# idthanm/env_build

Measured on AMD Instinct MI355X. Metric: env-steps/s (batched rollout) at N_env x N_veh; achieved HBM GB/s vs peak, higher is better.
Workload: dtype f32

## Files before the change

env_build_amd/csrc/eb_rollout.hip:

```cpp
#include <type_traits>

#include "eb_device.h"
#include "eb_kernels.h"

#pragma clang fp contract(off)

namespace eb {

typedef float f2u __attribute__((ext_vector_type(2), aligned(4)));
typedef float v2f __attribute__((ext_vector_type(2)));
EB_DEV v2f fma2(v2f a, v2f b, v2f c) { return __builtin_elementwise_fma(a, b, c); }

template <typename ST> struct Stored;
template <> struct Stored<float> {
    static EB_DEV f4u load4(const float* p) { return *reinterpret_cast<const f4u*>(p); }
    static EB_DEV float load1(const float* p) { return *p; }
    static EB_DEV void store4(float* p, f4u v) { *reinterpret_cast<f4u*>(p) = v; }
    static EB_DEV void store1(float* p, float v) { *p = v; }
    static EB_DEV float round(float v) { return v; }
    static EB_DEV void store4_wt(float* p, f4u v) { asm volatile("global_store_dwordx4 %0, %1, off sc1\n\ts_nop 1" :: "v"(p), "v"(v) : "memory"); }
    static EB_DEV void store1_wt(float* p, float v) { asm volatile("global_store_dword %0, %1, off sc1" :: "v"(p), "v"(v) : "memory"); }
};
typedef _Float16 h4u __attribute__((ext_vector_type(4), aligned(2)));
template <> struct Stored<_Float16> {
    static EB_DEV f4u load4(const _Float16* p) {
        const h4u h = *reinterpret_cast<const h4u*>(p);
        return f4u{(float)h.x, (float)h.y, (float)h.z, (float)h.w};
    }
    static EB_DEV float load1(const _Float16* p) { return (float)*p; }
    static EB_DEV void store4(_Float16* p, f4u v) {
        *reinterpret_cast<h4u*>(p) = h4u{(_Float16)v.x, (_Float16)v.y, (_Float16)v.z, (_Float16)v.w};
    }
    static EB_DEV void store1(_Float16* p, float v) { *p = (_Float16)v; }
    static EB_DEV float round(float v) { return (float)(_Float16)v; }
    static EB_DEV void store4_wt(_Float16* p, f4u v) {
        typedef unsigned u2v __attribute__((ext_vector_type(2)));
        const u2v bits = __builtin_bit_cast(u2v, h4u{(_Float16)v.x, (_Float16)v.y, (_Float16)v.z, (_Float16)v.w});
        asm volatile("global_store_dwordx2 %0, %1, off sc1" :: "v"(p), "v"(bits) : "memory");
    }
    static EB_DEV void store1_wt(_Float16* p, float v) {
        const unsigned bits = __builtin_bit_cast(unsigned short, (_Float16)v);
        asm volatile("global_store_short %0, %1, off sc1" :: "v"(p), "v"(bits) : "memory");
    }
};

EB_DEV void lds_barrier() { asm volatile("s_waitcnt lgkmcnt(0)\n\ts_barrier" ::: "memory"); }
typedef __attribute__((address_space(3))) int lds_int;
EB_DEV void lds_publish(int* flag, int value) {
    asm volatile("s_waitcnt lgkmcnt(0)" ::: "memory");
    *(volatile lds_int*)flag = value;
}
EB_DEV void lds_wait_until(int* flag, int value) {
    while (*(volatile lds_int*)flag != value) __builtin_amdgcn_s_sleep(2);
    asm volatile("" ::: "memory");
}

template <int CTRL, int ROW_MASK>
EB_DEV double dpp_f64(double v) {
    const unsigned long long b = __builtin_bit_cast(unsigned long long, v);
    const unsigned lo = (unsigned)__builtin_amdgcn_update_dpp(0, (int)(unsigned)b, CTRL, ROW_MASK, 0xf, false);
    const unsigned hi = (unsigned)__builtin_amdgcn_update_dpp(0, (int)(unsigned)(b >> 32), CTRL, ROW_MASK, 0xf, false);
    return __builtin_bit_cast(double, ((unsigned long long)hi << 32) | lo);
}
EB_DEV double wave_sum_f64(double v) {
    v += dpp_f64<0x111, 0xf>(v);
    v += dpp_f64<0x112, 0xf>(v);
    v += dpp_f64<0x114, 0xf>(v);
    v += dpp_f64<0x118, 0xf>(v);
    v += dpp_f64<0x142, 0xa>(v);
    v += dpp_f64<0x143, 0xc>(v);
    return v;
}
template <int CTRL, int ROW_MASK>
EB_DEV float dpp_max_f32(float v) {
    const float o = __builtin_bit_cast(float, __builtin_amdgcn_update_dpp(0, __builtin_bit_cast(int, v), CTRL, ROW_MASK, 0xf, false));
    return o > v ? o : v;
}
EB_DEV float wave_max_f32(float v) {
    v = dpp_max_f32<0x111, 0xf>(v);
    v = dpp_max_f32<0x112, 0xf>(v);
    v = dpp_max_f32<0x114, 0xf>(v);
    v = dpp_max_f32<0x118, 0xf>(v);
    v = dpp_max_f32<0x142, 0xa>(v);
    v = dpp_max_f32<0x143, 0xc>(v);
    return v;
}

EB_DEV void acc_record(double* recs, bool act, int lane, float v_r, float v_t, float v_p) {
    const double s_r = wave_sum_f64(act ? (double)v_r : 0.0);
    const double s_t = wave_sum_f64(act ? (double)v_t : 0.0);
    const double s_p = wave_sum_f64(act ? (double)v_p : 0.0);
    const unsigned long long any = __builtin_amdgcn_ballot_w64(act && v_p > 0.0f);
    if (lane == 63) {
        typedef double d2v __attribute__((ext_vector_type(2)));
        d2v* rec = reinterpret_cast<d2v*>(recs + (size_t)ACC_RECORD_DOUBLES * blockIdx.x);
        rec[0] = d2v{s_r, s_t};
        rec[1] = d2v{s_p, __builtin_bit_cast(double, any)};
    }
}

EB_DEV unsigned agent_load_u32(const unsigned* p) {
    unsigned v;
    asm volatile("global_load_dword %0, %1, off sc1\n\ts_waitcnt vmcnt(0)" : "=v"(v) : "v"(p) : "memory");
    return v;
}
EB_DEV unsigned long long agent_load_u64(const void* p) {
    unsigned long long v;
    asm volatile("global_load_dwordx2 %0, %1, off sc1\n\ts_waitcnt vmcnt(0)" : "=v"(v) : "v"(p) : "memory");
    return v;
}
EB_DEV void agent_store_u32(unsigned* p, unsigned v) { asm volatile("global_store_dword %0, %1, off sc1" :: "v"(p), "v"(v) : "memory"); }
EB_DEV void agent_add_u32(unsigned* p, unsigned v) { asm volatile("global_atomic_add %0, %1, off sc1" :: "v"(p), "v"(v) : "memory"); }

template <typename ST>
struct FusedHot {
    const ST* obs_in;
    ST* obs_out;
    int n_env, obs_dim, n_veh, envs_per_tile;
    unsigned nv_magic;
    int do_rewards;
    double* acc_rec;
    const unsigned char* turn;
    long long t_entry;
};
constexpr int HOT_REWARDS = 1, HOT_PRIO = 2;

template <typename ST>
EB_DEV int env_of_item(const FusedHot<ST>& H, int item) {
    return H.nv_magic ? (int)__umulhi((unsigned)item, H.nv_magic) : item;
}

#define EB_MARK(A, row, i) do { if ((A).trace && (threadIdx.x & 63) == 0) (A).trace[(size_t)(row) * 8 + (i)] = wall_clock64(); } while (0)
#define EB_MARK_PLACE(A, row) do { if ((A).trace && (threadIdx.x & 63) == 0) (A).trace[(size_t)(row) * 8 + 7] = \
    ((long long)__builtin_amdgcn_s_getreg((31 << 11) | 20) << 32) | (unsigned)__builtin_amdgcn_s_getreg((31 << 11) | 4); } while (0)

constexpr int QCAP = 160;
constexpr int TAPE_QCAP = 192;

template <int PRE = 3, bool COARSE = true>
EB_DEV int closest_cell_index(const FusedArgs& A, const float* xy10, const float* phi10, int p, int roff, float px, float py,
                              float& rx, float& ry, float& rphi) {
    const float* xy = xy10 + 2 * roff;
    const float* ph = phi10 + roff;
    const float fx = (px - A.gx0) * CELL_INV, fy = (py - A.gy0) * CELL_INV;
    unsigned c = 0xffffffffu;
    if (fx >= 0.0f && fx < (float)A.gnx && fy >= 0.0f && fy < (float)A.gny) c = A.cells[(p * A.gny + (int)fy) * A.gnx + (int)fx];
    if (c == 0xffffffffu) {
        int r_first = 0, r_last = 1 << 30;
        if constexpr (COARSE) {
            const PathTables& pt = *A.dt;
            int lo, hi, lo2, hi2;
            const int how = coarse_cell_ranges(pt, p, px, py, lo, hi, lo2, hi2);
            if (how == 1) return closest_in_ranges(xy, ph, lo, hi, lo2, hi2, px, py, rx, ry, rphi);
            if (how == 2) { r_first = lo; r_last = hi; }
        }
        const int n = p == 0 ? A.red_len[0] : p == 1 ? A.red_len[1] : A.red_len[2];
        const int bi = closest_reduced_index(reinterpret_cast<const float2*>(xy), A.rad_all + 32 * p, n, px, py, r_first, r_last);
        rx = xy[2 * bi]; ry = xy[2 * bi + 1]; rphi = ph[bi];
        return bi;
    }
    if (PRE > 0 && A.scan_one_trip) return closest_in_range<0>(xy, ph, (int)(c & 0xffffu), (int)(c >> 16), px, py, rx, ry, rphi);
    return closest_in_range<PRE>(xy, ph, (int)(c & 0xffffu), (int)(c >> 16), px, py, rx, ry, rphi);
}

template <int RW, int RPT>
struct FusedSmem {
    static constexpr int ITEMS = RW * 64 * RPT;
    float4 ego[64];
    unsigned char turn[64];
    unsigned long long mask[64];
    float2 pen[ITEMS];
    v2f qxy[RW][QCAP];
    v2f qsc[RW][QCAP];
    int qitem[RW][QCAP];
    int ego_ready;
    int waves_done;
};

template <int TASK, int RW, int RPT, typename ST>
EB_DEV void env_wave(const FusedHot<ST>& H, const FusedArgs& A, FusedSmem<RW, RPT>& S, int e0, int nE) {
    const int lane = threadIdx.x;
    const int D = H.obs_dim, NV = H.n_veh;
    const bool act = lane < nE;
    const int e = act ? lane : 0, ge = e0 + e;
    const ST* hin = H.obs_in + (size_t)ge * D;
    ST* hout = H.obs_out + (size_t)ge * D;

    const f4u h0 = Stored<ST>::load4(hin), h1 = Stored<ST>::load4(hin + 4);
    const float h8 = Stored<ST>::load1(hin + 8);
    const f2u araw = *reinterpret_cast<const f2u*>(A.actions + 2 * (size_t)ge);
    int p = A.path_id;
    if (A.training) {
        const int pr = A.ref_idx[ge];
        p = (pr >= 0 && pr < A.n_paths) ? pr : -1;
    }
    float sh_prev = 0.0f;
    if (A.shield_punish && !A.shield_first && act) sh_prev = A.shield_punish[ge];
    const int trow = blockIdx.x * (RW + 1);
    if (lane == 0) { S.ego_ready = 0; S.waves_done = 0; }
    lds_barrier();
    EB_MARK(A, trow, 0);
    EB_MARK_PLACE(A, trow);
    const bool do_rewards = (H.do_rewards & HOT_REWARDS) != 0;
    const float st[6] = {h0.x, h0.y, h0.z, h0.w, h1.x, h1.y};
    const float phi_rad = deg2rad(st[5]);
    float es, ec;
    sincos_det(phi_rad, es, ec);
    if (do_rewards) {
        S.ego[lane] = make_float4(st[3], st[4], es, ec);
        S.mask[lane] = 0ull;
        lds_publish(&S.ego_ready, 1);
        EB_MARK(A, trow, 1);
    }

    float steer, a_x;
    if (A.actions_raw) action_transform(araw.x, araw.y, steer, a_x);
    else { steer = araw.x; a_x = araw.y; }
    if (act && A.scaled_actions) *reinterpret_cast<f2u*>(A.scaled_actions + 2 * (size_t)ge) = f2u{steer, a_x};
    float rew = 0.0f;
    if (act && do_rewards) {
        const float punish_steer = -sq(steer), punish_a_x = -sq(a_x);
        const float punish_yaw_rate = -sq(st[2]);
        const float devi_y = -sq(h1.z);
        const float devi_phi = -sq(deg2rad(h1.w));
        const float devi_v = -sq(h8);
        rew = 0.05f * devi_v + 0.8f * devi_y + 30.0f * devi_phi + 0.02f * punish_yaw_rate +
              5.0f * punish_steer + 0.05f * punish_a_x;
        A.out5[ge] = rew;
    }
    float nx[6];
    f_xu_core(st, steer, a_x, TAU10, phi_rad, es, ec, nx);
    nx[0] = __builtin_fminf(__builtin_fmaxf(nx[0], 0.0f), 35.0f);
    float t0 = 0.0f, t1 = 0.0f, t2 = 0.0f;
    if (p >= 0) {
        const int roff = p == 0 ? A.red_off[0] : p == 1 ? A.red_off[1] : A.red_off[2];
        EB_MARK(A, trow, 2);
        float rx = 0.0f, ry = 0.0f, rphi = 0.0f;
        constexpr int SCAN_PRE = RW * RPT >= 32 ? 0 : 3;
        const int bi = closest_cell_index<SCAN_PRE>(A, A.xy10, A.phi10, p, roff, nx[3], nx[4], rx, ry, rphi);
        t0 = two2one<TASK>(nx[3], nx[4], rx, ry);
        if (A.trace) { asm volatile("" :: "v"(t0)); EB_MARK(A, trow, 3); }
        t1 = deal_with_phi_diff(nx[5] - rphi);
        t2 = nx[0] - EXP_V;
        if (A.n_future > 0 && act) {
            const PathTables& pt = *A.dt;
            const int len = pt.len[p];
            ST* otrk = hout + 9;
            int cur = bi * 10;
            for (int k = 0; k < A.n_future; ++k) {
                cur += 80;
                if (cur >= len - 2) cur = len - 2;
                const int fi = clamp_index(cur, len);
                Stored<ST>::store1(otrk + 3 * k, pt.x[p][fi] - nx[3]);
                Stored<ST>::store1(otrk + 3 * k + 1, pt.y[p][fi] - nx[4]);
                Stored<ST>::store1(otrk + 3 * k + 2, deal_with_phi_diff(nx[5] - pt.phi[p][fi]));
            }
        }
    } else if (A.n_future > 0 && act) {
        ST* otrk = hout + 9;
        for (int c = 0; c < 3 * A.n_future; ++c) Stored<ST>::store1(otrk + c, 0.0f);
    }
    if (act) {
        Stored<ST>::store4(hout, f4u{nx[0], nx[1], nx[2], nx[3]});
        Stored<ST>::store4(hout + 4, f4u{nx[4], nx[5], t0, t1});
        Stored<ST>::store1(hout + 8, t2);
    }
    EB_MARK(A, trow, 4);
    if (!do_rewards) return;
    float road_t = 0.0f, road_r = 0.0f;
    road_terms<TASK>(st[3] + LWS * ec, st[4] + LWS * es, road_t, road_r);
    road_terms<TASK>(st[3] - LWS * ec, st[4] - LWS * es, road_t, road_r);
    lds_wait_until(&S.waves_done, RW);
    EB_MARK(A, trow, 5);

    float pun_t = 0.0f, pun_r = 0.0f;
    if (act) {
        float a35 = 0.0f, a25 = 0.0f;
        unsigned long long m = S.mask[lane];
        while (m) {
            const int jj = __ffsll((long long)m) - 1;
            m &= m - 1;
            const float2 ps = S.pen[lane * NV + jj];
            a35 += ps.x;
            a25 += ps.y;
        }
        const size_t n = (size_t)H.n_env;
        pun_t = a35 + road_t;
        pun_r = a25 + road_r;
        A.out5[n + ge] = pun_t;
        A.out5[2 * n + ge] = pun_r;
        A.out5[3 * n + ge] = a25;
        A.out5[4 * n + ge] = road_r;
        if (A.shield_punish) {
            const float pacc = sh_prev + (A.shield_row == 3 ? a25 : pun_r);
            A.shield_punish[ge] = pacc;
            if (A.shield_last) A.shield_safe[ge] = pacc > 0.0f ? 0 : 1;
        }
    }
    if (H.acc_rec && A.acc_final) {
        acc_record(H.acc_rec, act, lane, rew, pun_t, pun_r);
        const float dy = __builtin_fabsf(Stored<ST>::round(t0));
        const double s_dy = wave_sum_f64(act ? (double)dy : 0.0);
        const float m_dy = wave_max_f32(act && dy > 0.0f ? dy : 0.0f);
        if (lane == 63) {
            typedef double d2v __attribute__((ext_vector_type(2)));
            reinterpret_cast<d2v*>(A.acc_final)[blockIdx.x] = d2v{s_dy, (double)m_dy};
        }
    }
    EB_MARK(A, trow, 6);
}

template <typename SM, typename ST>
EB_DEV void queue_terms(const FusedHot<ST>& H, SM& S, const float4* ego, int item, float x, float y, float vs, float vc) {
    const int e2 = env_of_item(H, item), j2 = item - e2 * H.n_veh;
    const float4 eg = ego[e2];
    float t35[4], t25[4];
    const float4 pts = make_float4(eg.x + LWS * eg.w, eg.y + LWS * eg.z, eg.x - LWS * eg.w, eg.y - LWS * eg.z);
    veh2veh_terms(pts, x, y, vs, vc, t35, t25);
    const float p35 = ((t35[0] + t35[1]) + t35[2]) + t35[3];
    const float p25 = ((t25[0] + t25[1]) + t25[2]) + t25[3];
    if (p35 != 0.0f) {
        S.pen[item] = make_float2(p35, p25);
        atomicOr(&S.mask[e2], 1ull << j2);
    }
}
template <typename SM, typename ST>
EB_DEV void queue_pass(const FusedHot<ST>& H, SM& S, const float4* ego, int w, int lane, int base, int n) {
    if (lane < n) {
        const v2f vxy = S.qxy[w][base + lane];
        float vs, vc;
        sincos_det(deg2rad(S.qphi[w][base + lane]), vs, vc);
        queue_terms(H, S, ego, S.qitem[w][base + lane], vxy.x, vxy.y, vs, vc);
    }
}
template <typename SM, typename ST>
EB_DEV void queue_pass_sc(const FusedHot<ST>& H, SM& S, const float4* ego, int w, int lane, int base, int n) {
    if (lane < n) {
        const v2f vxy = S.qxy[w][base + lane], sc = S.qsc[w][base + lane];
        queue_terms(H, S, ego, S.qitem[w][base + lane], vxy.x, vxy.y, sc.x, sc.y);
    }
}


template <int TASK, int RW, int RPT, bool FAST, int PF, typename ST>
EB_DEV void record_wave(const FusedHot<ST>& H, const FusedArgs& A, FusedSmem<RW, RPT>& S, int e0, int nE) {
    constexpr int RL = RW * 64;
    const int rtid = threadIdx.x - 64, w = rtid >> 6, lane = rtid & 63;
    const int NV = H.n_veh, D = H.obs_dim, HD = D - 4 * NV;
    const int items = nE * NV;
    const ST* tin = H.obs_in + (size_t)e0 * D;
    ST* tout = H.obs_out + (size_t)e0 * D;
    const int e_first = env_of_item(H, rtid), j_first = rtid - e_first * NV;
    const int epk = RL / NV;
    const int off_first = 4 * rtid + (e_first + 1) * HD, off_step = 4 * RL + epk * HD;
    auto item_of = [&](int k) { return k * RL + rtid; };
    auto env_of = [&](int k) { return FAST ? e_first + k * epk : env_of_item(H, item_of(k)); };
    auto off_of = [&](int k) { return FAST ? off_first + k * off_step : 4 * item_of(k) + (env_of(k) + 1) * HD; };

    static_assert(PF >= 1 && PF <= RPT, "record loads in flight per lane");
    const int turn_code = H.turn[lane];
    f4u rec[PF];
    const bool full_tile = items == RL * RPT;
    auto load_records = [&](auto full_tag) {
        constexpr bool FULL = decltype(full_tag)::value;
#pragma unroll
        for (int k = 0; k < PF; ++k) {
            const bool valid = FULL || item_of(k) < items;
            rec[k] = Stored<ST>::load4(tin + (valid ? off_of(k) : 4 * (items - 1) + nE * HD));
            if (!valid) rec[k].x = 1e30f;
        }
    };
    if (full_tile) load_records(std::true_type{}); else load_records(std::false_type{});
    const bool acc_prev = w == 0 && H.acc_rec && A.prev_out5;
    float pv_r = 0.0f, pv_t = 0.0f, pv_p = 0.0f;
    if (acc_prev && lane < nE) {
        const size_t n = (size_t)H.n_env;
        const float* po = A.prev_out5 + e0 + lane;
        pv_r = po[0]; pv_t = po[n]; pv_p = po[2 * n];
    }
    const int trow = blockIdx.x * (RW + 1) + 1 + w;
    lds_barrier();
    EB_MARK(A, trow, 0);
    EB_MARK_PLACE(A, trow);
    if (A.trace && lane == 0) A.trace[(size_t)trow * 8 + 6] = H.t_entry;
    const bool do_rewards = (H.do_rewards & HOT_REWARDS) != 0;
    const bool by_progress = (H.do_rewards & HOT_PRIO) != 0;
    S.turn[lane] = (unsigned char)turn_code;
    const TurnC tc_lane = turn_consts(S.turn[FAST ? j_first : 0]);
    const SinCosK SK = sincos_consts();

    int qn = 0;
    auto drain = [&]() {
        for (int base = 0; base < qn; base += 64) queue_pass_sc(H, S, S.ego, w, lane, base, min(64, qn - base));
        qn = 0;
    };
    auto near_test = [&](int item, const v2f eg, const f4u r, const v2f sc) {
        const v2f d = v2f{r.x, r.y} - eg;
        const v2f d2 = d * d;
        const bool near = d2.x + d2.y < 40.5f;
        const unsigned long long b = __builtin_amdgcn_ballot_w64(near);
        if (b) {
            if (near) {
                const int pos = (int)__builtin_amdgcn_mbcnt_hi((unsigned)(b >> 32), __builtin_amdgcn_mbcnt_lo((unsigned)b, (unsigned)qn));
                S.qxy[w][pos] = v2f{r.x, r.y};
                S.qsc[w][pos] = sc;
                S.qitem[w][pos] = item;
            }
            qn += __popcll(b);
        }
    };
    if (do_rewards) {
        lds_wait_until(&S.ego_ready, 1);
        EB_MARK(A, trow, 3);
    }
    const bool test_near = do_rewards;
    int k_late = test_near ? RPT : 0;
    auto main_loop = [&](auto full_tag) {
        constexpr bool FULL = decltype(full_tag)::value;
        v2f egoxy[RPT];
        if (test_near) {
#pragma unroll
            for (int k = 0; k < RPT; ++k) {
                const int item = k * RL + rtid;
                const int env = FAST ? e_first + k * epk : env_of_item(H, item);
                egoxy[k] = *reinterpret_cast<const v2f*>(&S.ego[(FULL || item < items) ? env : 0]);
            }
        }
#pragma unroll
        for (int k = 0; k < RPT; ++k) {
            int k_item = k * RL, k_env = k * epk, k_off = k * off_step;
            asm volatile("" : "+s"(k_item), "+s"(k_env), "+s"(k_off));
            const int item = k_item + rtid;
            const int env = FAST ? e_first + k_env : env_of_item(H, item);
            const int off = FAST ? off_first + k_off : 4 * item + (env + 1) * HD;
            const bool valid = FULL || item < items;
            const TurnC tc = FAST ? tc_lane : turn_consts(S.turn[valid ? item - env * NV : 0]);
            float sn, cs;
            if ((k * 4) % RPT == 0 && by_progress)
                switch (3 - (k * 4) / RPT) {
                    case 3: __builtin_amdgcn_s_setprio(3); break;
                    case 2: __builtin_amdgcn_s_setprio(2); break;
                    case 1: __builtin_amdgcn_s_setprio(1); break;
                    default: __builtin_amdgcn_s_setprio(0); break;
                }
            const f4u nv = predict_record_tc<ST>(rec[k % PF], tc, SK, sn, cs);
            if (k < k_late) {
                near_test(item, egoxy[k], rec[k % PF], v2f{sn, cs});
                if (qn > QCAP - 64) k_late = k + 1;
            }
            if (k + PF < RPT) {
                const bool v2 = FULL || item_of(k + PF) < items;
                rec[k % PF] = Stored<ST>::load4(tin + (v2 ? off_of(k + PF) : 4 * (items - 1) + nE * HD));
                if (!v2) rec[k % PF].x = 1e30f;
            }
            if (valid) Stored<ST>::store4(reinterpret_cast<ST*>(reinterpret_cast<char*>(tout) + (unsigned)off * (unsigned)sizeof(ST)), nv);
            if (k == 0) EB_MARK(A, trow, 1);
            if (k == RPT - 1) EB_MARK(A, trow, 2);
            if (k & 1) __builtin_amdgcn_sched_barrier(0);
        }
    };
    if (full_tile) main_loop(std::true_type{}); else main_loop(std::false_type{});
    if (!do_rewards) return;
    if (by_progress) __builtin_amdgcn_s_setprio(0);
    if (test_near && k_late < RPT) {
        for (int k = k_late; k < RPT; ++k) {
            drain();
            const bool valid = item_of(k) < items;
            f4u r = Stored<ST>::load4(tin + (valid ? off_of(k) : 4 * (items - 1) + nE * HD));
            if (!valid) r.x = 1e30f;
            float sn, cs;
            sincos_det(deg2rad(r.w), sn, cs);
            near_test(item_of(k), *reinterpret_cast<const v2f*>(&S.ego[valid ? env_of(k) : 0]), r, v2f{sn, cs});
        }
    }
    EB_MARK(A, trow, 4);
    drain();
    asm volatile("s_waitcnt lgkmcnt(0)" ::: "memory");
    if (lane == 0) atomicAdd(&S.waves_done, 1);
    if (acc_prev) {
        asm volatile("" : "+v"(pv_r), "+v"(pv_t), "+v"(pv_p));
        acc_record(A.prev_rec, lane < nE, lane, pv_r, pv_t, pv_p);
    }
    EB_MARK(A, trow, 5);
}

template <int RW, int RPT>
struct TapeSmem {
    static constexpr int ITEMS = RW * 64 * RPT;
    float4 ego[2][64];
    unsigned char turn[64];
    unsigned long long mask[64];
    float2 pen[ITEMS];
    v2f qxy[RW][TAPE_QCAP];
    float qphi[RW][TAPE_QCAP];
    int qitem[RW][TAPE_QCAP];
    int ego_ready;
    int waves_done;
    int pub_done;
    int abort;
};
EB_DEV bool lds_wait_or_abort(int* flag, int value, int* abort) {
    while (*(volatile lds_int*)flag < value) {
        if (*(volatile lds_int*)abort) return false;
        __builtin_amdgcn_s_sleep(2);
    }
    asm volatile("" ::: "memory");
    return true;
}

struct GateSmem {
    f2u act[2][64];
    float out5[2][5][64];
    float head[2][9][64];
    int bi[2][64];
    int act_ready;
    int out_ready;
    int sent;
};

template <typename ST, bool WT>
EB_DEV void store_head_row(const FusedArgs& A, ST* row, const float (&hv)[9], int bi, int p) {
    auto s4 = [&](ST* q, f4u v) { if (WT) Stored<ST>::store4_wt(q, v); else Stored<ST>::store4(q, v); };
    auto s1 = [&](ST* q, float v) { if (WT) Stored<ST>::store1_wt(q, v); else Stored<ST>::store1(q, v); };
    s4(row, f4u{hv[0], hv[1], hv[2], hv[3]});
    s4(row + 4, f4u{hv[4], hv[5], hv[6], hv[7]});
    s1(row + 8, hv[8]);
    ST* otrk = row + 9;
    if (p >= 0) {
        const PathTables& pt = *A.dt;
        const int len = pt.len[p];
        int cur = bi * 10;
        for (int k = 0; k < A.n_future; ++k) {
            cur += 80;
            if (cur >= len - 2) cur = len - 2;
            const int fi = clamp_index(cur, len);
            s1(otrk + 3 * k, pt.x[p][fi] - hv[3]);
            s1(otrk + 3 * k + 1, pt.y[p][fi] - hv[4]);
            s1(otrk + 3 * k + 2, deal_with_phi_diff(hv[5] - pt.phi[p][fi]));
        }
    } else {
        for (int c = 0; c < 3 * A.n_future; ++c) s1(otrk + c, 0.0f);
    }
}

EB_DEV int env_path(const FusedArgs& A, int ge) {
    if (!A.training) return A.path_id;
    const int pr = A.ref_idx[ge];
    return (pr >= 0 && pr < A.n_paths) ? pr : -1;
}

template <int RW, int RPT>
EB_DEV void in_courier(const FusedArgs& A, TapeSmem<RW, RPT>& S, GateSmem& G, int e0, int nE, int n_env, int horizon) {
    const int lane = threadIdx.x & 63;
    const int ge = e0 + (lane < nE ? lane : 0);
    for (int t = 0; t < horizon; ++t) {
        if (t >= 2 && !lds_wait_or_abort(&G.out_ready, t - 1, &S.abort)) return;
        unsigned open = agent_load_u32(A.gate_ready + t);
        if (!open && t >= 1 && !lds_wait_or_abort(&G.out_ready, t, &S.abort)) return;
        for (int spins = 0; !open && spins <= A.gate_spin; ++spins) {
            open = agent_load_u32(A.gate_ready + t);
            if (open || *(volatile lds_int*)&S.abort) break;
            __builtin_amdgcn_s_sleep(4);
        }
        if (!open) {
            if (lane == 0) agent_store_u32(A.gate_status, 1u);
            lds_publish(&S.abort, 1);
            return;
        }
        const unsigned long long bits = agent_load_u64(A.actions + 2 * ((size_t)t * n_env + ge));
        G.act[t & 1][lane] = __builtin_bit_cast(f2u, bits);
        lds_publish(&G.act_ready, t + 1);
    }
}

template <int RW, int RPT, typename ST>
EB_DEV void out_courier(const FusedHot<ST>& H, const FusedArgs& A, TapeSmem<RW, RPT>& S, GateSmem& G, int e0, int nE, int horizon) {
    const int lane = threadIdx.x & 63;
    const bool act = lane < nE;
    const int ge = e0 + (act ? lane : 0);
    const size_t n = (size_t)H.n_env;
    const int p = env_path(A, ge);
    for (int t = 0; t < horizon; ++t) {
        if (!lds_wait_or_abort(&G.out_ready, t + 1, &S.abort)) return;
        if (act) {
            float* out5 = A.out5 + (size_t)t * 5 * n + ge;
#pragma unroll
            for (int c = 0; c < 5; ++c) Stored<float>::store1_wt(out5 + c * n, G.out5[t & 1][c][lane]);
            if (A.gate_obs) {
                float hv[9];
#pragma unroll
                for (int c = 0; c < 9; ++c) hv[c] = G.head[t & 1][c][lane];
                store_head_row<ST, true>(A, reinterpret_cast<ST*>(A.gate_obs) + ((size_t)t * n + ge) * H.obs_dim, hv, G.bi[t & 1][lane], p);
            }
        }
        asm volatile("s_waitcnt vmcnt(0)" ::: "memory");
        if (A.gate_obs && !lds_wait_or_abort(&S.pub_done, RW * (t + 1), &S.abort)) return;
        if (lane < 4) {
            typedef unsigned u4w __attribute__((ext_vector_type(4)));
            const u4w ones = {1u, 1u, 1u, 1u};
            unsigned* rec = A.gate_done + ((size_t)t * gridDim.x + blockIdx.x) * 16 + 4 * lane;
            asm volatile("global_store_dwordx4 %0, %1, off sc1\n\ts_nop 1" :: "v"(rec), "v"(ones) : "memory");
        }
        lds_publish(&G.sent, t + 1);
    }
}

template <int TASK, int RW, int RPT, bool GATED, typename ST>
EB_DEV void env_wave_tape(const FusedHot<ST>& H, const FusedArgs& A, TapeSmem<RW, RPT>& S, GateSmem* Gp, int e0, int nE, int horizon,
                          const float* xy10, const float* phi10) {
    const int lane = threadIdx.x;
    const int D = H.obs_dim, NV = H.n_veh;
    const bool act = lane < nE;
    const int e = act ? lane : 0, ge = e0 + e;
    const ST* hin = H.obs_in + (size_t)ge * D;
    ST* hout = H.obs_out + (size_t)ge * D;
    const f4u h0 = Stored<ST>::load4(hin), h1 = Stored<ST>::load4(hin + 4);
    float st[6] = {h0.x, h0.y, h0.z, h0.w, h1.x, h1.y};
    float trk[3] = {h1.z, h1.w, Stored<ST>::load1(hin + 8)};
    const int p = env_path(A, ge);
    const int roff = p == 1 ? A.red_off[1] : p == 2 ? A.red_off[2] : A.red_off[0];
    const size_t n = (size_t)H.n_env;
    constexpr bool gated = GATED;
    f2u araw = f2u{0.0f, 0.0f};
    if (!gated) araw = *reinterpret_cast<const f2u*>(A.actions + 2 * (size_t)ge);
    const int trow = blockIdx.x * (RW + 1);
    long long waited = 0;
    EB_MARK(A, trow, 0);
    for (int t = 0; t < horizon; ++t) {
        float* out5 = A.out5 + (size_t)t * 5 * n;
        f2u araw_next = araw;
        if (gated) {
            if (!lds_wait_or_abort(&Gp->act_ready, t + 1, &S.abort)) return;
            araw = Gp->act[t & 1][lane];
            if (t >= 2 && !lds_wait_or_abort(&Gp->sent, t - 1, &S.abort)) return;
        } else if (t + 1 < horizon) {
            araw_next = *reinterpret_cast<const f2u*>(A.actions + 2 * ((size_t)(t + 1) * n + ge));
        }
        const float phi_rad = deg2rad(st[5]);
        float es, ec;
        sincos_det(phi_rad, es, ec);
        S.ego[t & 1][lane] = make_float4(st[3], st[4], es, ec);
        S.mask[lane] = 0ull;
        lds_publish(&S.ego_ready, t + 1);
        float steer, a_x;
        action_transform(araw.x, araw.y, steer, a_x);
        auto put = [&](int c, float v) { if (gated) Gp->out5[t & 1][c][lane] = v; else out5[(size_t)c * n + ge] = v; };
        if (act) {
            const float punish_steer = -sq(steer), punish_a_x = -sq(a_x);
            const float punish_yaw_rate = -sq(st[2]);
            const float devi_y = -sq(trk[0]);
            const float devi_phi = -sq(deg2rad(trk[1]));
            const float devi_v = -sq(trk[2]);
            put(0, 0.05f * devi_v + 0.8f * devi_y + 30.0f * devi_phi + 0.02f * punish_yaw_rate +
                   5.0f * punish_steer + 0.05f * punish_a_x);
        }
        float nx[6];
        f_xu_core(st, steer, a_x, TAU10, phi_rad, es, ec, nx);
        nx[0] = __builtin_fminf(__builtin_fmaxf(nx[0], 0.0f), 35.0f);
        float t0 = 0.0f, t1 = 0.0f, t2 = 0.0f;
        int bi = 0;
        if (p >= 0) {
            float rx = 0.0f, ry = 0.0f, rphi = 0.0f;
            bi = closest_cell_index<0, false>(A, xy10, phi10, p, roff, nx[3], nx[4], rx, ry, rphi);
            t0 = two2one<TASK>(nx[3], nx[4], rx, ry);
            t1 = deal_with_phi_diff(nx[5] - rphi);
            t2 = nx[0] - EXP_V;
        }
        const float hv[9] = {nx[0], nx[1], nx[2], nx[3], nx[4], nx[5], t0, t1, t2};
        if (t == horizon - 1 && act) store_head_row<ST, false>(A, hout, hv, bi, p);
        if (GATED && A.gate_obs) {
#pragma unroll
            for (int c = 0; c < 9; ++c) Gp->head[t & 1][c][lane] = hv[c];
            Gp->bi[t & 1][lane] = bi;
        }
        float road_t = 0.0f, road_r = 0.0f;
        road_terms<TASK>(st[3] + LWS * ec, st[4] + LWS * es, road_t, road_r);
        road_terms<TASK>(st[3] - LWS * ec, st[4] - LWS * es, road_t, road_r);
        const long long w0 = A.trace ? wall_clock64() : 0;
        if (GATED) { if (!lds_wait_or_abort(&S.waves_done, RW * (t + 1), &S.abort)) return; }
        else lds_wait_until(&S.waves_done, RW * (t + 1));
        if (A.trace) waited += wall_clock64() - w0;
        if (act) {
            float a35 = 0.0f, a25 = 0.0f;
            unsigned long long m = S.mask[lane];
            while (m) {
                const int jj = __ffsll((long long)m) - 1;
                m &= m - 1;
                const float2 ps = S.pen[lane * NV + jj];
                a35 += ps.x;
                a25 += ps.y;
            }
            put(1, a35 + road_t);
            put(2, a25 + road_r);
            put(3, a25);
            put(4, road_r);
        }
        if (gated) lds_publish(&Gp->out_ready, t + 1);
#pragma unroll
        for (int c = 0; c < 6; ++c) st[c] = Stored<ST>::round(nx[c]);
        trk[0] = Stored<ST>::round(t0); trk[1] = Stored<ST>::round(t1); trk[2] = Stored<ST>::round(t2);
        araw = araw_next;
    }
    EB_MARK(A, trow, 1);
    if (A.trace && lane == 0) A.trace[(size_t)trow * 8 + 2] = waited;
}

template <int TASK, int RW, int RPT, bool FAST, bool GATED, typename ST>
EB_DEV void record_wave_tape(const FusedHot<ST>& H, const FusedArgs& A, TapeSmem<RW, RPT>& S, int e0, int nE, int horizon) {
    constexpr int RL = RW * 64;
    const int rtid = threadIdx.x - 64, w = rtid >> 6, lane = rtid & 63;
    const int NV = H.n_veh, D = H.obs_dim, HD = D - 4 * NV;
    const int items = nE * NV;
    const ST* tin = H.obs_in + (size_t)e0 * D;
    ST* tout = H.obs_out + (size_t)e0 * D;
    const int e_first = env_of_item(H, rtid), j_first = rtid - e_first * NV;
    const int epk = RL / NV;
    const int off_first = 4 * rtid + (e_first + 1) * HD, off_step = 4 * RL + epk * HD;
    auto item_of = [&](int k) { return k * RL + rtid; };
    auto env_of = [&](int k) { return FAST ? e_first + k * epk : env_of_item(H, item_of(k)); };
    auto off_of = [&](int k) { return FAST ? off_first + k * off_step : 4 * item_of(k) + (env_of(k) + 1) * HD; };
    const int turn_code = A.dt->turn[lane];
    f4u rec[RPT];
#pragma unroll
    for (int k = 0; k < RPT; ++k) {
        const bool valid = item_of(k) < items;
        rec[k] = Stored<ST>::load4(tin + (valid ? off_of(k) : 4 * (items - 1) + nE * HD));
        if (!valid) rec[k].x = 1e30f;
    }
    S.turn[lane] = (unsigned char)turn_code;
    const TurnC tc_lane = turn_consts(S.turn[FAST ? j_first : 0]);
    const SinCosK SK = sincos_consts();
    const int trow = blockIdx.x * (RW + 1) + 1 + w;
    long long waited = 0;
    EB_MARK(A, trow, 0);
    for (int t = 0; t < horizon; ++t) {
        const float4* ego = S.ego[t & 1];
        int qn = 0;
        auto drain = [&]() {
            for (int base = 0; base < qn; base += 64) queue_pass(H, S, ego, w, lane, base, min(64, qn - base));
            qn = 0;
        };
        const long long w0 = A.trace ? wall_clock64() : 0;
        if (GATED) { if (!lds_wait_or_abort(&S.ego_ready, t + 1, &S.abort)) return; }
        else lds_wait_until(&S.ego_ready, t + 1);
        if (A.trace) waited += wall_clock64() - w0;
#pragma unroll
        for (int k = 0; k < RPT; ++k) {
            int k_item = k * RL, k_env = k * epk;
            asm volatile("" : "+s"(k_item), "+s"(k_env));
            const int item = k_item + rtid;
            const int env = FAST ? e_first + k_env : env_of_item(H, item);
            if (k > 0 && (k & 1) == 0 && qn > 64) drain();
            const float4 eg = ego[item < items ? env : 0];
            const v2f d = v2f{rec[k].x, rec[k].y} - v2f{eg.x, eg.y};
            const v2f d2 = d * d;
            const bool near = d2.x + d2.y < 40.5f;
            const unsigned long long b = __builtin_amdgcn_ballot_w64(near);
            if (b) {
                if (near) {
                    const int pos = (int)__builtin_amdgcn_mbcnt_hi((unsigned)(b >> 32), __builtin_amdgcn_mbcnt_lo((unsigned)b, (unsigned)qn));
                    S.qxy[w][pos] = v2f{rec[k].x, rec[k].y};
                    S.qphi[w][pos] = rec[k].w;
                    S.qitem[w][pos] = item;
                }
                qn += __popcll(b);
            }
        }
        drain();
        asm volatile("s_waitcnt lgkmcnt(0)" ::: "memory");
        if (lane == 0) atomicAdd(&S.waves_done, 1);
#pragma unroll
        for (int k = 0; k < RPT; ++k) {
            int k_item = k * RL, k_env = k * epk;
            asm volatile("" : "+s"(k_item), "+s"(k_env));
            const int item = k_item + rtid;
            if (item < items) {
                const int env = FAST ? e_first + k_env : env_of_item(H, item);
                const TurnC tc = FAST ? tc_lane : turn_consts(S.turn[item - env * NV]);
                float sn_, cs_;
                const f4u nv = predict_record_tc<ST>(rec[k], tc, SK, sn_, cs_);
                rec[k] = f4u{Stored<ST>::round(nv.x), Stored<ST>::round(nv.y), Stored<ST>::round(nv.z), Stored<ST>::round(nv.w)};
                if (GATED && A.gate_obs) Stored<ST>::store4_wt(reinterpret_cast<ST*>(A.gate_obs) + ((size_t)t * H.n_env + e0) * D + off_of(k), rec[k]);
            }
            if (k & 1) __builtin_amdgcn_sched_barrier(0);
        }
        if (GATED && A.gate_obs) {
            asm volatile("s_waitcnt vmcnt(0)" ::: "memory");
            if (lane == 0) atomicAdd(&S.pub_done, 1);
        }
    }
#pragma unroll
    for (int k = 0; k < RPT; ++k)
        if (item_of(k) < items) Stored<ST>::store4(tout + off_of(k), rec[k]);
    EB_MARK(A, trow, 1);
    if (A.trace && lane == 0) A.trace[(size_t)trow * 8 + 2] = waited;
}

template <int TASK, int RW, int RPT, bool FAST, bool GATED, typename ST>
EB_DEV void tape_body(const FusedHot<ST>& H, const FusedArgs& A, int horizon) {
    __shared__ TapeSmem<RW, RPT> S;
    extern __shared__ __attribute__((aligned(16))) float staged[];
    const int e0 = blockIdx.x * H.envs_per_tile;
    const int nE = min(H.envs_per_tile, H.n_env - e0);
    __shared__ std::conditional_t<GATED, GateSmem, int> Gs;
    GateSmem* Gp = GATED ? reinterpret_cast<GateSmem*>(&Gs) : nullptr;
    if (threadIdx.x == 0) {
        S.ego_ready = 0; S.waves_done = 0; S.pub_done = 0; S.abort = 0;
        if (GATED) { Gp->act_ready = 0; Gp->out_ready = 0; Gp->sent = 0; }
    }
    const float* xy10 = A.xy10;
    const float* phi10 = A.phi10;
    if (A.stage_entries > 0) {
        const int n_xy = 2 * A.stage_entries, n_all = 3 * A.stage_entries;
        for (int i = threadIdx.x; i < n_all; i += (RW + (GATED ? 3 : 1)) * 64) staged[i] = i < n_xy ? A.xy10[i] : A.phi10[i - n_xy];
        xy10 = staged;
        phi10 = staged + n_xy;
    }
    lds_barrier();
    if (threadIdx.x < 64) {
        __builtin_amdgcn_s_setprio(3);
        env_wave_tape<TASK, RW, RPT, GATED, ST>(H, A, S, Gp, e0, nE, horizon, xy10, phi10);
    }
    else if (threadIdx.x < (RW + 1) * 64) record_wave_tape<TASK, RW, RPT, FAST, GATED, ST>(H, A, S, e0, nE, horizon);
    else if (GATED && threadIdx.x < (RW + 2) * 64) in_courier<RW, RPT>(A, S, *Gp, e0, nE, H.n_env, horizon);
    else if (GATED) out_courier<RW, RPT, ST>(H, A, S, *Gp, e0, nE, horizon);
}

template <int TASK, int RW, int RPT, bool FAST, int PF, typename ST>
EB_DEV void fused_body(const FusedHot<ST>& H, const FusedArgs& A) {
    __shared__ FusedSmem<RW, RPT> S;
    const int e0 = blockIdx.x * H.envs_per_tile;
    const int nE = min(H.envs_per_tile, H.n_env - e0);
    if (RW * RPT >= 32) asm volatile("; keep v79 allocated" ::: "v79");
    if (threadIdx.x < 64) {
        __builtin_amdgcn_s_setprio(2);
        env_wave<TASK, RW, RPT, ST>(H, A, S, e0, nE);
    } else {
        record_wave<TASK, RW, RPT, FAST, PF, ST>(H, A, S, e0, nE);
    }
}

#define EB_FUSED_KERNEL(NAME, RW, RPT, WAVES, VGPRS)                                                     \
    template <int TASK, bool FAST, int PF, typename ST>                                                  \
    __global__ __launch_bounds__((RW + 1) * 64, WAVES) __attribute__((amdgpu_num_vgpr(VGPRS))) void NAME( \
        const ST* obs_in, ST* obs_out, int n_env, int obs_dim, int n_veh, int envs_per_tile,             \
        unsigned nv_magic, int do_rewards, double* acc_rec, const unsigned char* turn_tab, const FusedArgs A) { \
        const FusedHot<ST> H{obs_in, obs_out, n_env, obs_dim, n_veh, envs_per_tile, nv_magic, do_rewards, acc_rec, turn_tab, \
                             wall_clock64()};                                                            \
        fused_body<TASK, RW, RPT, FAST, PF, ST>(H, A);                                                   \
    }
EB_FUSED_KERNEL(rollout_fused_4x8, 4, 8, 6, 80)
EB_FUSED_KERNEL(rollout_fused_4x4, 4, 4, 6, 80)
EB_FUSED_KERNEL(rollout_fused_1x4, 1, 4, 6, 80)

#define EB_TAPE_KERNEL(NAME, RW, RPT, GATED, WAVES)                                                      \
    template <int TASK, bool FAST, typename ST>                                                          \
    __global__ __launch_bounds__((RW + (GATED ? 3 : 1)) * 64, WAVES) void NAME(                          \
        const ST* obs_in, ST* obs_out, int n_env, int obs_dim, int n_veh, int envs_per_tile,             \
        unsigned nv_magic, int horizon, const FusedArgs A) {                                             \
        const FusedHot<ST> H{obs_in, obs_out, n_env, obs_dim, n_veh, envs_per_tile, nv_magic, HOT_REWARDS, nullptr, nullptr, 0ll}; \
        tape_body<TASK, RW, RPT, FAST, GATED, ST>(H, A, horizon);                                        \
    }
EB_TAPE_KERNEL(rollout_tape_4x8, 4, 8, false, 6)
EB_TAPE_KERNEL(rollout_tape_4x4, 4, 4, false, 1)
EB_TAPE_KERNEL(rollout_tape_1x4, 1, 4, false, 1)
EB_TAPE_KERNEL(rollout_gated_4x8, 4, 8, true, 4)
EB_TAPE_KERNEL(rollout_gated_4x4, 4, 4, true, 1)
EB_TAPE_KERNEL(rollout_gated_1x4, 1, 4, true, 1)

int tape_tile_variant(int variant, int n_veh, int storage_f16) {
    (void)storage_f16;
    return (variant == 0 && (4 * 64) % n_veh != 0) ? 1 : variant;
}

int fused_tile_records(int variant) {
    switch (variant) {
        case 0: return 4 * 64 * 8;
        case 1: return 4 * 64 * 4;
        default: return 1 * 64 * 4;
    }
}

int tape_blocks_per_cu(int task, int variant, int n_veh, int storage_f16, size_t dyn_bytes) {
    (void)task;
    const int rw = variant == 0 || variant == 1 ? 4 : 1;
    int nb = 0;
    const hipError_t e = with_bool(storage_f16, [&](auto f16) { return with_bool((rw * 64) % n_veh == 0, [&](auto fast) {
        using ST = std::conditional_t<f16, _Float16, float>;
        auto occ = [&](auto kernel) { return hipOccupancyMaxActiveBlocksPerMultiprocessor(&nb, kernel, (rw + 3) * 64, dyn_bytes); };
        return variant == 0 ? occ(rollout_gated_4x8<TASK_LEFT, fast, ST>) : variant == 1 ? occ(rollout_gated_4x4<TASK_LEFT, fast, ST>)
                                                                          : occ(rollout_gated_1x4<TASK_LEFT, fast, ST>);
    }); });
    return e == hipSuccess ? nb : 0;
}

typedef unsigned u4v __attribute__((ext_vector_type(4)));
__global__ __launch_bounds__(256) void gate_feed_kernel(int horizon, unsigned n_blocks, size_t step_words, const u4v* __restrict__ staged,
                                                        u4v* live, unsigned* gate_ready, const unsigned* gate_done,
                                                        unsigned* status, int spin) {
    constexpr int PRE = 8;
    for (int t = 0; t < horizon; ++t) {
        const u4v* src = staged + (size_t)t * step_words;
        u4v* dst = live + (size_t)t * step_words;
        u4v pre[PRE];
#pragma unroll
        for (int k = 0; k < PRE; ++k) {
            const size_t i = threadIdx.x + (size_t)k * blockDim.x;
            pre[k] = src[i < step_words ? i : 0];
        }
        int good = 1;
        if (t > 0) {
            for (unsigned b = threadIdx.x; b < n_blocks && good; b += blockDim.x) {
                const unsigned* w = gate_done + ((size_t)(t - 1) * n_blocks + b) * 16;
                for (int spins = 0; !agent_load_u32(w); ++spins) {
                    if (spins >= spin || ((spins & 31) == 31 && agent_load_u32(status))) { good = 0; break; }
                    __builtin_amdgcn_s_sleep(2);
                }
            }
        }
        if (!__syncthreads_and(good)) {
            if (threadIdx.x == 0) agent_store_u32(status + 1, 1u);
            return;
        }
#pragma unroll
        for (int k = 0; k < PRE; ++k) {
            const size_t i = threadIdx.x + (size_t)k * blockDim.x;
            if (i < step_words) asm volatile("global_store_dwordx4 %0, %1, off sc1\n\ts_nop 1" :: "v"(dst + i), "v"(pre[k]) : "memory");
        }
        for (size_t i = threadIdx.x + (size_t)PRE * blockDim.x; i < step_words; i += blockDim.x) {
            const u4v v = src[i];
            asm volatile("global_store_dwordx4 %0, %1, off sc1\n\ts_nop 1" :: "v"(dst + i), "v"(v) : "memory");
        }
        asm volatile("s_waitcnt vmcnt(0)" ::: "memory");
        __syncthreads();
        if (threadIdx.x == 0) agent_store_u32(gate_ready + t, 1u);
    }
}

hipError_t launch_gate_feed(int horizon, int n_blocks, size_t step_bytes, const void* staged, void* live,
                            unsigned* gate_ready, const unsigned* gate_done, unsigned* status, int spin, hipStream_t s) {
    hipLaunchKernelGGL(gate_feed_kernel, dim3(1), dim3(256), 0, s, horizon, (unsigned)n_blocks, step_bytes / 16,
                       reinterpret_cast<const u4v*>(staged), reinterpret_cast<u4v*>(live), gate_ready, gate_done, status, spin);
    return hipGetLastError();
}

static FusedArgs trace_checked(const FusedArgs& A_in, int grid, int waves_per_block) {
    FusedArgs A = A_in;
    if (A.trace && A.trace_words < (long long)grid * waves_per_block * 8) A.trace = nullptr;
    return A;
}

hipError_t launch_rollout_tape_fused(int task, int variant, const FusedArgs& A_in, int horizon, int grid, hipStream_t s) {
    const int rw = variant == 0 || variant == 1 ? 4 : 1;
    const FusedArgs A = trace_checked(A_in, grid, rw + 1);
    const bool gated = A.gate_ready != nullptr, fast = (rw * 64) % A.n_veh == 0;
    if (variant == 0 && !gated && !fast) return hipErrorInvalidValue;
    const dim3 g(grid), b((rw + 1 + (gated ? 2 : 0)) * 64);
    const size_t dyn = (size_t)A.stage_entries * 12;
    with_task(task, [&](auto t) { with_bool(A.storage_f16, [&](auto f16) { with_bool(fast, [&](auto fast_c) {
        using ST = std::conditional_t<f16, _Float16, float>;
        auto go = [&](auto kernel) {
            hipLaunchKernelGGL(kernel, g, b, dyn, s, reinterpret_cast<const ST*>(A.obs_in), reinterpret_cast<ST*>(A.obs_out), A.n_env,
                               A.obs_dim, A.n_veh, A.envs_per_tile, A.nv_magic, horizon, A);
        };
        if (gated && variant == 0) go(rollout_gated_4x8<t, fast_c, ST>);
        else if (gated && variant == 1) go(rollout_gated_4x4<t, fast_c, ST>);
        else if (gated) go(rollout_gated_1x4<t, fast_c, ST>);
        else if (variant == 0) go(rollout_tape_4x8<t, true, ST>);
        else if (variant == 1) go(rollout_tape_4x4<t, fast_c, ST>);
        else go(rollout_tape_1x4<t, fast_c, ST>);
    }); }); });
    return hipGetLastError();
}

hipError_t launch_rollout_fused(int task, int variant, const FusedArgs& A_in, int grid, hipStream_t s) {
    const int rw = variant == 0 || variant == 1 ? 4 : 1;
    const FusedArgs A = trace_checked(A_in, grid, rw + 1);
    const dim3 g(grid), b((rw + 1) * 64);
    const int hot = (A.do_rewards ? HOT_REWARDS : 0) | (A.by_progress ? HOT_PRIO : 0);
    const unsigned char* turn_tab = reinterpret_cast<const unsigned char*>(A.dt) + offsetof(PathTables, turn);
    with_task(task, [&](auto t) { with_bool(A.storage_f16, [&](auto f16) { with_bool((rw * 64) % A.n_veh == 0, [&](auto fast) {
        using ST = std::conditional_t<f16, _Float16, float>;
        auto go = [&](auto kernel) {
            hipLaunchKernelGGL(kernel, g, b, 0, s, reinterpret_cast<const ST*>(A.obs_in), reinterpret_cast<ST*>(A.obs_out), A.n_env,
                               A.obs_dim, A.n_veh, A.envs_per_tile, A.nv_magic, hot, A.acc_rec, turn_tab, A);
        };
        if (variant == 0 && A.rolling) go(rollout_fused_4x8<t, fast, 3, ST>);
        else if (variant == 0) go(rollout_fused_4x8<t, fast, 8, ST>);
        else if (variant == 1) go(rollout_fused_4x4<t, fast, 4, ST>);
        else go(rollout_fused_1x4<t, fast, 4, ST>);
    }); }); });
    return hipGetLastError();
}

}
```

Measured before the change: 4.508 billion.

## Precompute reward-store pointers, pack queue words, pipeline penalty loads, skip clock read

Several micro-optimizations land together in the fused rollout kernel. Reward output row pointers and shield parameters are hoisted into scalar registers before the LDS wait, and stores go through global address-space pointers with a byte offset. The penalty accumulation loop is software-pipelined so the next LDS load is issued before the current one is added. Queue items are packed with env and slot indices to avoid a magic-number division per queue entry, record prediction uses precomputed reciprocal constants, and the entry wall-clock read is skipped unless tracing is enabled. The packed queue word limits item, env and slot field widths, which could break at larger sizes.

```diff
diff --git a/env_build_amd/csrc/eb_rollout.hip b/env_build_amd/csrc/eb_rollout.hip
--- a/env_build_amd/csrc/eb_rollout.hip
+++ b/env_build_amd/csrc/eb_rollout.hip
@@ -46,6 +46,9 @@
 
 EB_DEV void lds_barrier() { asm volatile("s_waitcnt lgkmcnt(0)\n\ts_barrier" ::: "memory"); }
 typedef __attribute__((address_space(3))) int lds_int;
+typedef __attribute__((address_space(1))) float g_float;
+typedef __attribute__((address_space(1))) char g_char;
+typedef __attribute__((address_space(1))) unsigned char g_uchar;
 EB_DEV void lds_publish(int* flag, int value) {
     asm volatile("s_waitcnt lgkmcnt(0)" ::: "memory");
     *(volatile lds_int*)flag = value;
@@ -123,7 +126,7 @@
     const unsigned char* turn;
     long long t_entry;
 };
-constexpr int HOT_REWARDS = 1, HOT_PRIO = 2;
+constexpr int HOT_REWARDS = 1, HOT_PRIO = 2, HOT_TRACE = 4;
 
 template <typename ST>
 EB_DEV int env_of_item(const FusedHot<ST>& H, int item) {
@@ -270,6 +273,20 @@
     float road_t = 0.0f, road_r = 0.0f;
     road_terms<TASK>(st[3] + LWS * ec, st[4] + LWS * es, road_t, road_r);
     road_terms<TASK>(st[3] - LWS * ec, st[4] - LWS * es, road_t, road_r);
+    const size_t n = (size_t)H.n_env;
+    char* row1 = reinterpret_cast<char*>(A.out5 + n);
+    char* row2 = reinterpret_cast<char*>(A.out5 + 2 * n);
+    char* row3 = reinterpret_cast<char*>(A.out5 + 3 * n);
+    char* row4 = reinterpret_cast<char*>(A.out5 + 4 * n);
+    float* sh_punish = A.shield_punish;
+    unsigned char* sh_safe = A.shield_safe;
+    int sh_row = A.shield_row, sh_last = A.shield_last;
+    double* acc_final = H.acc_rec ? A.acc_final : nullptr;
+    unsigned ge_bytes = (unsigned)ge * 4u;
+    int pen_row = lane * NV;
+    asm volatile("" : "+v"(road_t), "+v"(road_r), "+v"(ge_bytes), "+v"(pen_row));
+    asm volatile("" : "+s"(row1), "+s"(row2), "+s"(row3), "+s"(row4));
+    asm volatile("" : "+s"(sh_punish), "+s"(sh_safe), "+s"(sh_row), "+s"(sh_last), "+s"(acc_final));
     lds_wait_until(&S.waves_done, RW);
     EB_MARK(A, trow, 5);
 
@@ -277,27 +294,32 @@
     if (act) {
         float a35 = 0.0f, a25 = 0.0f;
         unsigned long long m = S.mask[lane];
-        while (m) {
-            const int jj = __ffsll((long long)m) - 1;
+        if (m) {
+            float2 ps = S.pen[pen_row + __ffsll((long long)m) - 1];
             m &= m - 1;
-            const float2 ps = S.pen[lane * NV + jj];
+            while (m) {
+                const float2 nxt = S.pen[pen_row + __ffsll((long long)m) - 1];
+                m &= m - 1;
+                a35 += ps.x;
+                a25 += ps.y;
+                ps = nxt;
+            }
             a35 += ps.x;
             a25 += ps.y;
         }
-        const size_t n = (size_t)H.n_env;
         pun_t = a35 + road_t;
         pun_r = a25 + road_r;
-        A.out5[n + ge] = pun_t;
-        A.out5[2 * n + ge] = pun_r;
-        A.out5[3 * n + ge] = a25;
-        A.out5[4 * n + ge] = road_r;
-        if (A.shield_punish) {
-            const float pacc = sh_prev + (A.shield_row == 3 ? a25 : pun_r);
-            A.shield_punish[ge] = pacc;
-            if (A.shield_last) A.shield_safe[ge] = pacc > 0.0f ? 0 : 1;
-        }
-    }
-    if (H.acc_rec && A.acc_final) {
+        *(g_float*)((g_char*)row1 + ge_bytes) = pun_t;
+        *(g_float*)((g_char*)row2 + ge_bytes) = pun_r;
+        *(g_float*)((g_char*)row3 + ge_bytes) = a25;
+        *(g_float*)((g_char*)row4 + ge_bytes) = road_r;
+        if (sh_punish) {
+            const float pacc = sh_prev + (sh_row == 3 ? a25 : pun_r);
+            *(g_float*)((g_char*)sh_punish + ge_bytes) = pacc;
+            if (sh_last) ((g_uchar*)sh_safe)[ge] = pacc > 0.0f ? 0 : 1;
+        }
+    }
+    if (acc_final) {
         acc_record(H.acc_rec, act, lane, rew, pun_t, pun_r);
         const float dy = __builtin_fabsf(Stored<ST>::round(t0));
         const double s_dy = wave_sum_f64(act ? (double)dy : 0.0);
@@ -310,9 +332,12 @@
     EB_MARK(A, trow, 6);
 }
 
-template <typename SM, typename ST>
-EB_DEV void queue_terms(const FusedHot<ST>& H, SM& S, const float4* ego, int item, float x, float y, float vs, float vc) {
-    const int e2 = env_of_item(H, item), j2 = item - e2 * H.n_veh;
+constexpr int QW_ITEM_BITS = 11, QW_ENV_BITS = 6;
+EB_DEV int queue_word(int item, int env, int slot) { return item | (env << QW_ITEM_BITS) | (slot << (QW_ITEM_BITS + QW_ENV_BITS)); }
+template <typename SM>
+EB_DEV void queue_terms(SM& S, const float4* ego, int qw, float x, float y, float vs, float vc) {
+    const int item = qw & ((1 << QW_ITEM_BITS) - 1), e2 = (qw >> QW_ITEM_BITS) & ((1 << QW_ENV_BITS) - 1);
+    const int j2 = (int)((unsigned)qw >> (QW_ITEM_BITS + QW_ENV_BITS));
     const float4 eg = ego[e2];
     float t35[4], t25[4];
     const float4 pts = make_float4(eg.x + LWS * eg.w, eg.y + LWS * eg.z, eg.x - LWS * eg.w, eg.y - LWS * eg.z);
@@ -324,23 +349,44 @@
         atomicOr(&S.mask[e2], 1ull << j2);
     }
 }
-template <typename SM, typename ST>
-EB_DEV void queue_pass(const FusedHot<ST>& H, SM& S, const float4* ego, int w, int lane, int base, int n) {
+template <typename SM>
+EB_DEV void queue_pass(SM& S, const float4* ego, int w, int lane, int base, int n) {
     if (lane < n) {
         const v2f vxy = S.qxy[w][base + lane];
         float vs, vc;
         sincos_det(deg2rad(S.qphi[w][base + lane]), vs, vc);
-        queue_terms(H, S, ego, S.qitem[w][base + lane], vxy.x, vxy.y, vs, vc);
-    }
-}
-template <typename SM, typename ST>
-EB_DEV void queue_pass_sc(const FusedHot<ST>& H, SM& S, const float4* ego, int w, int lane, int base, int n) {
+        queue_terms(S, ego, S.qitem[w][base + lane], vxy.x, vxy.y, vs, vc);
+    }
+}
+template <typename SM>
+EB_DEV void queue_pass_sc(SM& S, const float4* ego, int w, int lane, int base, int n) {
     if (lane < n) {
         const v2f vxy = S.qxy[w][base + lane], sc = S.qsc[w][base + lane];
-        queue_terms(H, S, ego, S.qitem[w][base + lane], vxy.x, vxy.y, sc.x, sc.y);
-    }
-}
-
+        queue_terms(S, ego, S.qitem[w][base + lane], vxy.x, vxy.y, sc.x, sc.y);
+    }
+}
+
+
+struct RecK { double r180, rpi, r10; float pi, npi; };
+EB_DEV RecK rec_consts() {
+    RecK k{1.0 / (double)C180::value, 1.0 / (double)CPi::value, 1.0 / (double)C10::value, PI_F, -PI_F};
+    asm volatile("" : "+s"(k.r180), "+s"(k.rpi), "+s"(k.r10), "+s"(k.pi), "+s"(k.npi));
+    return k;
+}
+EB_DEV f4u predict_record_k(const f4u rec, const TurnC tc, const SinCosK K, const RecK R, float& sn_out, float& cs_out) {
+    const float v = rec.z;
+    const float v10 = div_by(v, R.r10);
+    const float phi_rad = div_by(rec.w * PI_F, R.r180);
+    sincos_det_k(phi_rad, K, sn_out, cs_out);
+    const float nx_ = rec.x + v10 * cs_out, ny_ = rec.y + v10 * sn_out;
+    const bool middle = (rec.x > -HALF_CROSS && rec.x < HALF_CROSS) && (rec.y > -HALF_CROSS && rec.y < HALF_CROSS);
+    const float u10 = div_by(div_by(v, tc.rc), R.r10);
+    const float dphi = (middle && tc.enabled != 0.0f) ? u10 : 0.0f;
+    float nphi = phi_rad + dphi;
+    if (nphi > R.pi) nphi = nphi - TWO_PI_F;
+    if (nphi <= R.npi) nphi = nphi + TWO_PI_F;
+    return f4u{nx_, ny_, v, div_by(nphi * 180.0f, R.rpi)};
+}
 
 template <int TASK, int RW, int RPT, bool FAST, int PF, typename ST>
 EB_DEV void record_wave(const FusedHot<ST>& H, const FusedArgs& A, FusedSmem<RW, RPT>& S, int e0, int nE) {
@@ -388,13 +434,15 @@
     S.turn[lane] = (unsigned char)turn_code;
     const TurnC tc_lane = turn_consts(S.turn[FAST ? j_first : 0]);
     const SinCosK SK = sincos_consts();
+    const RecK RK = rec_consts();
+    const int qw_first = queue_word(rtid, e_first, j_first);
 
     int qn = 0;
     auto drain = [&]() {
-        for (int base = 0; base < qn; base += 64) queue_pass_sc(H, S, S.ego, w, lane, base, min(64, qn - base));
+        for (int base = 0; base < qn; base += 64) queue_pass_sc(S, S.ego, w, lane, base, min(64, qn - base));
         qn = 0;
     };
-    auto near_test = [&](int item, const v2f eg, const f4u r, const v2f sc) {
+    auto near_test = [&](int item, int env, int k_word, const v2f eg, const f4u r, const v2f sc) {
         const v2f d = v2f{r.x, r.y} - eg;
         const v2f d2 = d * d;
         const bool near = d2.x + d2.y < 40.5f;
@@ -404,7 +452,7 @@
                 const int pos = (int)__builtin_amdgcn_mbcnt_hi((unsigned)(b >> 32), __builtin_amdgcn_mbcnt_lo((unsigned)b, (unsigned)qn));
                 S.qxy[w][pos] = v2f{r.x, r.y};
                 S.qsc[w][pos] = sc;
-                S.qitem[w][pos] = item;
+                S.qitem[w][pos] = FAST ? qw_first + k_word : queue_word(item, env, item - env * NV);
             }
             qn += __popcll(b);
         }
@@ -443,9 +491,9 @@
                     case 1: __builtin_amdgcn_s_setprio(1); break;
                     default: __builtin_amdgcn_s_setprio(0); break;
                 }
-            const f4u nv = predict_record_tc<ST>(rec[k % PF], tc, SK, sn, cs);
+            const f4u nv = predict_record_k(rec[k % PF], tc, SK, RK, sn, cs);
             if (k < k_late) {
-                near_test(item, egoxy[k], rec[k % PF], v2f{sn, cs});
+                near_test(item, env, k_item + (k_env << QW_ITEM_BITS), egoxy[k], rec[k % PF], v2f{sn, cs});
                 if (qn > QCAP - 64) k_late = k + 1;
             }
             if (k + PF < RPT) {
@@ -470,7 +518,7 @@
             if (!valid) r.x = 1e30f;
             float sn, cs;
             sincos_det(deg2rad(r.w), sn, cs);
-            near_test(item_of(k), *reinterpret_cast<const v2f*>(&S.ego[valid ? env_of(k) : 0]), r, v2f{sn, cs});
+            near_test(item_of(k), env_of(k), k * RL + ((k * epk) << QW_ITEM_BITS), *reinterpret_cast<const v2f*>(&S.ego[valid ? env_of(k) : 0]), r, v2f{sn, cs});
         }
     }
     EB_MARK(A, trow, 4);
@@ -730,6 +778,7 @@
     S.turn[lane] = (unsigned char)turn_code;
     const TurnC tc_lane = turn_consts(S.turn[FAST ? j_first : 0]);
     const SinCosK SK = sincos_consts();
+    const int qw_first = queue_word(rtid, e_first, j_first);
     const int trow = blockIdx.x * (RW + 1) + 1 + w;
     long long waited = 0;
     EB_MARK(A, trow, 0);
@@ -737,7 +786,7 @@
         const float4* ego = S.ego[t & 1];
         int qn = 0;
         auto drain = [&]() {
-            for (int base = 0; base < qn; base += 64) queue_pass(H, S, ego, w, lane, base, min(64, qn - base));
+            for (int base = 0; base < qn; base += 64) queue_pass(S, ego, w, lane, base, min(64, qn - base));
             qn = 0;
         };
         const long long w0 = A.trace ? wall_clock64() : 0;
@@ -761,7 +810,7 @@
                     const int pos = (int)__builtin_amdgcn_mbcnt_hi((unsigned)(b >> 32), __builtin_amdgcn_mbcnt_lo((unsigned)b, (unsigned)qn));
                     S.qxy[w][pos] = v2f{rec[k].x, rec[k].y};
                     S.qphi[w][pos] = rec[k].w;
-                    S.qitem[w][pos] = item;
+                    S.qitem[w][pos] = FAST ? qw_first + k_item + (k_env << QW_ITEM_BITS) : queue_word(item, env, item - env * NV);
                 }
                 qn += __popcll(b);
             }
@@ -846,7 +895,7 @@
         const ST* obs_in, ST* obs_out, int n_env, int obs_dim, int n_veh, int envs_per_tile,             \
         unsigned nv_magic, int do_rewards, double* acc_rec, const unsigned char* turn_tab, const FusedArgs A) { \
         const FusedHot<ST> H{obs_in, obs_out, n_env, obs_dim, n_veh, envs_per_tile, nv_magic, do_rewards, acc_rec, turn_tab, \
-                             wall_clock64()};                                                            \
+                             (do_rewards & HOT_TRACE) ? wall_clock64() : 0ll};                                                            \
         fused_body<TASK, RW, RPT, FAST, PF, ST>(H, A);                                                   \
     }
 EB_FUSED_KERNEL(rollout_fused_4x8, 4, 8, 6, 80)
@@ -977,7 +1026,7 @@
     const int rw = variant == 0 || variant == 1 ? 4 : 1;
     const FusedArgs A = trace_checked(A_in, grid, rw + 1);
     const dim3 g(grid), b((rw + 1) * 64);
-    const int hot = (A.do_rewards ? HOT_REWARDS : 0) | (A.by_progress ? HOT_PRIO : 0);
+    const int hot = (A.do_rewards ? HOT_REWARDS : 0) | (A.by_progress ? HOT_PRIO : 0) | (A.trace ? HOT_TRACE : 0);
     const unsigned char* turn_tab = reinterpret_cast<const unsigned char*>(A.dt) + offsetof(PathTables, turn);
     with_task(task, [&](auto t) { with_bool(A.storage_f16, [&](auto f16) { with_bool((rw * 64) % A.n_veh == 0, [&](auto fast) {
         using ST = std::conditional_t<f16, _Float16, float>;
```

Result: no change. 4.492 billion (median of 2 runs) (-0.4%).
